# manikya7022/Continual-Learning-for-Dynamic-Video-Quality-Enhancement

Hardware: AMD Instinct MI355X
Metric: train frames/sec (2x SR, T=3, 540p->1080p) (higher is better)
Workload: dtype bf16

## Files before the change

### continual-learning-for-dynamic-video-quality-enhancement_amd/csrc/corr_mfma.hip

```cpp
#include <type_traits>
#include "common.h"

namespace nvq {

constexpr int MT_H = 8, MT_W = 16;
constexpr int MD = 4, MN = 9;
constexpr int MHH = MT_H + 2 * MD;
constexpr int MHW = MT_W + 2 * MD;
constexpr int MHP = MHH * MHW;
constexpr int M_T = 512;
constexpr int M_DSTR = 96;
constexpr int M_OSTR = 84;

typedef unsigned m_u32x4 __attribute__((ext_vector_type(4)));
typedef short m_s16x4 __attribute__((ext_vector_type(4)));

__device__ __forceinline__ unsigned pack_bf16x2(float lo, float hi) {
    typedef __bf16 b2 __attribute__((ext_vector_type(2)));
    const b2 v = {(__bf16)lo, (__bf16)hi};
    return __builtin_bit_cast(unsigned, v);
}
__device__ __forceinline__ m_u32x4 cvt_f8_bf16(float4 a, float4 b) {
    return (m_u32x4){pack_bf16x2(a.x, a.y), pack_bf16x2(a.z, a.w), pack_bf16x2(b.x, b.y), pack_bf16x2(b.z, b.w)};
}

template <int C, int YS>
__device__ __forceinline__ void m_stage_halo(const float* __restrict__ src, int ld, int n, int H, int W, int ty0, int tx0,
                                             __bf16* ys, int src_bf16) {
    constexpr int PPP = C / 8;
    constexpr int ITEMS = MHP * PPP;
    constexpr int PER = ITEMS / M_T;
    static_assert(ITEMS % M_T == 0, "halo pieces must divide evenly");
    if (src_bf16) {
        const __bf16* s16 = reinterpret_cast<const __bf16*>(src);
        m_u32x4 v[PER];
        unsigned okm = 0;
#pragma unroll
        for (int k = 0; k < PER; ++k) {
            const int item = threadIdx.x + k * M_T;
            const int hp = item / PPP, q = item - hp * PPP;
            const int hy = hp / MHW, hx = hp - hy * MHW;
            const int gy = ty0 + hy - MD, gx = tx0 + hx - MD;
            const bool ok = gy >= 0 && gy < H && gx >= 0 && gx < W;
            okm |= (ok ? 1u : 0u) << k;
            v[k] = *reinterpret_cast<const m_u32x4*>(s16 + (ok ? ((size_t)(n * H + gy) * W + gx) * ld + 8 * q : 0));
        }
#pragma unroll
        for (int k = 0; k < PER; ++k) {
            const int item = threadIdx.x + k * M_T;
            const int hp = item / PPP, q = item - hp * PPP;
            *reinterpret_cast<m_u32x4*>(ys + hp * YS + 8 * q) = (okm >> k) & 1 ? v[k] : (m_u32x4){0u, 0u, 0u, 0u};
        }
        return;
    }
    float4 a[PER], b[PER];
    unsigned okm = 0;
#pragma unroll
    for (int k = 0; k < PER; ++k) {
        const int item = threadIdx.x + k * M_T;
        const int hp = item / PPP, q = item - hp * PPP;
        const int hy = hp / MHW, hx = hp - hy * MHW;
        const int gy = ty0 + hy - MD, gx = tx0 + hx - MD;
        const bool ok = gy >= 0 && gy < H && gx >= 0 && gx < W;
        okm |= (ok ? 1u : 0u) << k;
        const float* p = src + (ok ? ((size_t)(n * H + gy) * W + gx) * ld + 8 * q : 0);
        a[k] = ld4(p);
        b[k] = ld4(p + 4);
    }
#pragma unroll
    for (int k = 0; k < PER; ++k) {
        const int item = threadIdx.x + k * M_T;
        const int hp = item / PPP, q = item - hp * PPP;
        const m_u32x4 v = cvt_f8_bf16(a[k], b[k]);
        *reinterpret_cast<m_u32x4*>(ys + hp * YS + 8 * q) = (okm >> k) & 1 ? v : (m_u32x4){0u, 0u, 0u, 0u};
    }
}

template <int C, bool OUT_BF16>
__global__ __launch_bounds__(M_T) void corr_fwd_mfma_kernel(const float* __restrict__ x1, int x1_ld,
                                                            const float* __restrict__ x2, int x2_ld, int x2_images, int H,
                                                            int W, int tilesX, int tilesY, float* __restrict__ out,
                                                            int out_ld, int in_bf16) {
    constexpr int YS = OUT_BF16 ? C + 8 : C + 16;
    constexpr int KS = C / 32;
    typedef typename std::conditional<OUT_BF16, __bf16, float>::type stage_t;
    __shared__ __attribute__((aligned(16))) __bf16 ys[MHP * YS];
    __shared__ __attribute__((aligned(16))) stage_t stage[MT_H * MT_W * M_OSTR];
    int bt = xcd_tile(blockIdx.x, gridDim.x);
    const int tx = bt % tilesX; bt /= tilesX;
    const int ty = bt % tilesY;
    const int n = bt / tilesY;
    const int lane = threadIdx.x & 63, r = threadIdx.x >> 6;
    const int p = lane & 15, g = lane >> 4;
    const int gy = ty * MT_H + r, gx = tx * MT_W + p;
    const bool inside = gy < H && gx < W;

    bf16x8 xb[KS];
    {
        const size_t off = inside ? ((size_t)(n * H + gy) * W + gx) * x1_ld : 0;
#pragma unroll
        for (int s = 0; s < KS; ++s) {
            if (in_bf16) {
                m_u32x4 v = *reinterpret_cast<const m_u32x4*>(reinterpret_cast<const __bf16*>(x1) + off + 32 * s + 8 * g);
                if (!inside) v = (m_u32x4){0u, 0u, 0u, 0u};
                xb[s] = __builtin_bit_cast(bf16x8, v);
            } else {
                float4 a = ld4(x1 + off + 32 * s + 8 * g), b = ld4(x1 + off + 32 * s + 8 * g + 4);
                if (!inside) { a = make_float4(0.f, 0.f, 0.f, 0.f); b = a; }
                xb[s] = __builtin_bit_cast(bf16x8, cvt_f8_bf16(a, b));
            }
        }
    }
    m_stage_halo<C, YS>(x2, x2_ld, n % x2_images, H, W, ty * MT_H, tx * MT_W, ys, in_bf16);
    stage_t* srow = stage + (r * MT_W) * M_OSTR;
    if (lane < 16) { srow[lane * M_OSTR + 81] = (stage_t)0.f; srow[lane * M_OSTR + 82] = (stage_t)0.f; srow[lane * M_OSTR + 83] = (stage_t)0.f; }
    __syncthreads();

    const float inv = 1.f / (float)C;
#pragma unroll 1
    for (int i = 0; i < MN; ++i) {
#pragma unroll
        for (int qb = 0; qb < 2; ++qb) {
            f32x4 acc = {0.f, 0.f, 0.f, 0.f};
            const __bf16* arow = ys + ((r + i) * MHW + qb * 8 + p) * YS + 8 * g;
#pragma unroll
            for (int s = 0; s < KS; ++s)
                acc = __builtin_amdgcn_mfma_f32_16x16x32_bf16(*reinterpret_cast<const bf16x8*>(arow + 32 * s), xb[s], acc, 0,
                                                              0, 0);
#pragma unroll
            for (int e = 0; e < 4; ++e) {
                const int m = 4 * g + e;
                const int j = qb * 8 + m - p;
                if (j >= 0 && j <= 8 && (qb == 0 || m >= 8)) srow[p * M_OSTR + i * MN + j] = (stage_t)(acc[e] * inv);
            }
        }
    }
    __syncthreads();
    if (gy >= H) return;
    if constexpr (OUT_BF16) {
        __bf16* o16 = reinterpret_cast<__bf16*>(out);
        const int ppp = out_ld / 8;
        for (int item = lane; item < MT_W * ppp; item += 64) {
            const int px = item / ppp, q = item - px * ppp;
            if (tx * MT_W + px >= W) continue;
            typedef unsigned u2 __attribute__((ext_vector_type(2)));
            u2 lo = {0u, 0u}, hi = {0u, 0u};
            if (8 * q < M_OSTR) lo = *reinterpret_cast<const u2*>(srow + px * M_OSTR + 8 * q);
            if (8 * q + 4 < M_OSTR) hi = *reinterpret_cast<const u2*>(srow + px * M_OSTR + 8 * q + 4);
            *reinterpret_cast<m_u32x4*>(o16 + ((size_t)(n * H + gy) * W + tx * MT_W + px) * out_ld + 8 * q) =
                (m_u32x4){lo[0], lo[1], hi[0], hi[1]};
        }
    } else {
        const int ppp = out_ld / 4;
        for (int item = lane; item < MT_W * ppp; item += 64) {
            const int px = item / ppp, q = item - px * ppp;
            if (tx * MT_W + px >= W) continue;
            float4 v = make_float4(0.f, 0.f, 0.f, 0.f);
            if (4 * q < M_OSTR) v = ld4(srow + px * M_OSTR + 4 * q);
            st4(out + ((size_t)(n * H + gy) * W + tx * MT_W + px) * out_ld + 4 * q, v);
        }
    }
}

constexpr int MS_SEG = 4;
constexpr int MS_MAXWG = 512;

template <int C, bool OUT_BF16>
__global__ __launch_bounds__(M_T) void corr_fwd_strip_kernel(const __bf16* __restrict__ x1, int x1_ld,
                                                             const __bf16* __restrict__ x2, int x2_ld, int x2_images, int H,
                                                             int W, int tilesX, int tilesY, int njobs,
                                                             float* __restrict__ out, int out_ld) {
    constexpr int YS = OUT_BF16 ? C + 8 : C + 16;
    constexpr int KS = C / 32;
    constexpr int PPP = C / 8;
    constexpr int HITEMS = 8 * MHW * PPP;
    constexpr int HPER = (HITEMS + M_T - 1) / M_T;
    typedef typename std::conditional<OUT_BF16, __bf16, float>::type stage_t;
    __shared__ __attribute__((aligned(16))) __bf16 ys[MHP * YS];
    __shared__ __attribute__((aligned(16))) stage_t stage[MT_H * MT_W * M_OSTR];
    const int tid = threadIdx.x;
    const int lane = tid & 63, r = tid >> 6;
    const int p = lane & 15, g = lane >> 4;
    stage_t* srow = stage + (r * MT_W) * M_OSTR;
    if (lane < 16) { srow[lane * M_OSTR + 81] = (stage_t)0.f; srow[lane * M_OSTR + 82] = (stage_t)0.f; srow[lane * M_OSTR + 83] = (stage_t)0.f; }
    const float inv = 1.f / (float)C;
    const int seg_rows = (tilesY + MS_SEG - 1) / MS_SEG;

    m_u32x4 hv[HPER], xv[KS];
    unsigned hokm = 0;
    bool xin = false;
    auto fetch_rows = [&](int n2, int ty, int tx, int half) {
        hokm = 0;
        int tid_o = tid;
        asm volatile("" : "+v"(tid_o));
#pragma unroll
        for (int k = 0; k < HPER; ++k) {
            const int item = tid_o + k * M_T;
            const int hp = item / PPP, q = item - hp * PPP;
            const int hyl = hp / MHW, hx = hp - hyl * MHW;
            const int gy = ty * MT_H + 8 * half + hyl - MD, gx = tx * MT_W + hx - MD;
            const bool ok = item < HITEMS && gy >= 0 && gy < H && gx >= 0 && gx < W;
            hokm |= (ok ? 1u : 0u) << k;
            hv[k] = *reinterpret_cast<const m_u32x4*>(x2 + (ok ? ((size_t)(n2 * H + gy) * W + gx) * x2_ld + 8 * q : 0));
        }
    };
    auto commit_rows = [&](int ty, int half) {
#pragma unroll
        for (int k = 0; k < HPER; ++k) {
            const int item = tid + k * M_T;
            const int hp = item / PPP, q = item - hp * PPP;
            const int hyl = hp / MHW, hx = hp - hyl * MHW;
            const int slot = (8 * half + hyl + 8 * (ty & 1)) & 15;
            if (item < HITEMS)
                *reinterpret_cast<m_u32x4*>(ys + (slot * MHW + hx) * YS + 8 * q) = (hokm >> k) & 1 ? hv[k] : (m_u32x4){0u, 0u, 0u, 0u};
        }
    };
    auto fetch_x1 = [&](int n, int ty, int tx) {
        const int gy = ty * MT_H + r, gx = tx * MT_W + p;
        xin = gy < H && gx < W;
        const size_t off = xin ? ((size_t)(n * H + gy) * W + gx) * x1_ld : 0;
#pragma unroll
        for (int s2 = 0; s2 < KS; ++s2) xv[s2] = *reinterpret_cast<const m_u32x4*>(x1 + off + 32 * s2 + 8 * g);
    };

    for (int job = blockIdx.x; job < njobs; job += gridDim.x) {
        int jt = job;
        const int seg = jt % MS_SEG; jt /= MS_SEG;
        const int tx = jt % tilesX;
        const int n = jt / tilesX;
        const int n2 = n % x2_images;
        const int ty0 = seg * seg_rows, ty1 = min(ty0 + seg_rows, tilesY);
        if (ty0 >= ty1) continue;
        __syncthreads();
        fetch_rows(n2, ty0, tx, 0);
        commit_rows(ty0, 0);
        fetch_rows(n2, ty0, tx, 1);
        fetch_x1(n, ty0, tx);
        for (int ty = ty0; ty < ty1; ++ty) {
            bf16x8 xb[KS];
            commit_rows(ty, 1);
#pragma unroll
            for (int s2 = 0; s2 < KS; ++s2) xb[s2] = __builtin_bit_cast(bf16x8, xin ? xv[s2] : (m_u32x4){0u, 0u, 0u, 0u});
            __syncthreads();
            if (ty + 1 < ty1) { fetch_rows(n2, ty + 1, tx, 1); fetch_x1(n, ty + 1, tx); }
            const int rot = 8 * (ty & 1);
#pragma unroll 1
            for (int i = 0; i < MN; ++i) {
#pragma unroll
                for (int qb = 0; qb < 2; ++qb) {
                    f32x4 acc = {0.f, 0.f, 0.f, 0.f};
                    const __bf16* arow = ys + ((((r + i) + rot) & 15) * MHW + qb * 8 + p) * YS + 8 * g;
#pragma unroll
                    for (int s2 = 0; s2 < KS; ++s2)
                        acc = __builtin_amdgcn_mfma_f32_16x16x32_bf16(*reinterpret_cast<const bf16x8*>(arow + 32 * s2), xb[s2], acc,
                                                                      0, 0, 0);
#pragma unroll
                    for (int e = 0; e < 4; ++e) {
                        const int m = 4 * g + e;
                        const int j = qb * 8 + m - p;
                        if (j >= 0 && j <= 8 && (qb == 0 || m >= 8)) srow[p * M_OSTR + i * MN + j] = (stage_t)(acc[e] * inv);
                    }
                }
            }
            const int gy = ty * MT_H + r;
            if (gy < H) {
                if constexpr (OUT_BF16) {
                    __bf16* o16 = reinterpret_cast<__bf16*>(out);
                    const int ppp = out_ld / 8;
                    for (int item = lane; item < MT_W * ppp; item += 64) {
                        const int px = item / ppp, q = item - px * ppp;
                        if (tx * MT_W + px >= W) continue;
                        typedef unsigned u2 __attribute__((ext_vector_type(2)));
                        u2 lo = {0u, 0u}, hi = {0u, 0u};
                        if (8 * q < M_OSTR) lo = *reinterpret_cast<const u2*>(srow + px * M_OSTR + 8 * q);
                        if (8 * q + 4 < M_OSTR) hi = *reinterpret_cast<const u2*>(srow + px * M_OSTR + 8 * q + 4);
                        *reinterpret_cast<m_u32x4*>(o16 + ((size_t)(n * H + gy) * W + tx * MT_W + px) * out_ld + 8 * q) =
                            (m_u32x4){lo[0], lo[1], hi[0], hi[1]};
                    }
                } else {
                    const int ppp = out_ld / 4;
                    for (int item = lane; item < MT_W * ppp; item += 64) {
                        const int px = item / ppp, q = item - px * ppp;
                        if (tx * MT_W + px >= W) continue;
                        float4 v = make_float4(0.f, 0.f, 0.f, 0.f);
                        if (4 * q < M_OSTR) v = ld4(srow + px * M_OSTR + 4 * q);
                        st4(out + ((size_t)(n * H + gy) * W + tx * MT_W + px) * out_ld + 4 * q, v);
                    }
                }
            }
            __syncthreads();
        }
    }
}

template <int C, int WHICH, bool D_BF16>
__global__ __launch_bounds__(M_T) void corr_bwd_mfma_kernel(const float* __restrict__ dcorr, int dcorr_ld,
                                                            const float* __restrict__ other, int other_ld,
                                                            int other_images, int H, int W, int tilesX, int tilesY,
                                                            float* __restrict__ dx, int dx_ld, int dx_coff,
                                                            int accumulate, int other_bf16, int groups, int group_images,
                                                            __bf16* __restrict__ dx16, int dx16_ld, const nvq_corr_addends ad) {
    constexpr int YS = WHICH == 1 ? C + 8 : C + 16;
    constexpr int NCB = C / 16;
    constexpr int DPX = WHICH == 1 ? MT_H * MT_W : MHP;
    __shared__ __attribute__((aligned(16))) __bf16 ys[MHP * YS];
    __shared__ __attribute__((aligned(16))) __bf16 ds[DPX * M_DSTR];
    int bt = xcd_tile(blockIdx.x, gridDim.x);
    const int tx = bt % tilesX; bt /= tilesX;
    const int ty = bt % tilesY;
    const int n0 = bt / tilesY;
    const int lane = threadIdx.x & 63, r = threadIdx.x >> 6;
    const int p = lane & 15, g = lane >> 4;
    f32x4 acc[NCB];
#pragma unroll
    for (int cb = 0; cb < NCB; ++cb) acc[cb] = (f32x4){0.f, 0.f, 0.f, 0.f};
#pragma unroll 1
    for (int gi = 0; gi < groups; ++gi) {
    const int n = n0 + gi * group_images;
    if (gi > 0) __syncthreads();

    {
        constexpr int ITEMS = DPX * 12;
        constexpr int PER = (ITEMS + M_T - 1) / M_T;
        const __bf16* d16 = reinterpret_cast<const __bf16*>(dcorr);
        if constexpr (D_BF16) {
            m_u32x4 v[PER];
            unsigned okm = 0;
#pragma unroll
            for (int k = 0; k < PER; ++k) {
                const int item = threadIdx.x + k * M_T;
                const int dp = item / 12, q = item - dp * 12;
                int gy, gx;
                if (WHICH == 1) { gy = ty * MT_H + dp / MT_W; gx = tx * MT_W + dp % MT_W; }
                else { gy = ty * MT_H + dp / MHW - MD; gx = tx * MT_W + dp % MHW - MD; }
                const bool ok = item < ITEMS && gy >= 0 && gy < H && gx >= 0 && gx < W;
                okm |= (ok ? 1u : 0u) << k;
                v[k] = *reinterpret_cast<const m_u32x4*>(d16 + (ok ? ((size_t)(n * H + gy) * W + gx) * dcorr_ld + 8 * q : 0));
            }
#pragma unroll
            for (int k = 0; k < PER; ++k) {
                const int item = threadIdx.x + k * M_T;
                const int dp = item / 12, q = item - dp * 12;
                if (item < ITEMS)
                    *reinterpret_cast<m_u32x4*>(ds + dp * M_DSTR + 8 * q) = (okm >> k) & 1 ? v[k] : (m_u32x4){0u, 0u, 0u, 0u};
            }
        } else {
#pragma unroll 3
            for (int k = 0; k < PER; ++k) {
                const int item = threadIdx.x + k * M_T;
                if (item >= ITEMS) break;
                const int dp = item / 12, q = item - dp * 12;
                int gy, gx;
                if (WHICH == 1) { gy = ty * MT_H + dp / MT_W; gx = tx * MT_W + dp % MT_W; }
                else { gy = ty * MT_H + dp / MHW - MD; gx = tx * MT_W + dp % MHW - MD; }
                const bool ok = gy >= 0 && gy < H && gx >= 0 && gx < W;
                m_u32x4 v = {0u, 0u, 0u, 0u};
                if (ok) {
                    const size_t idx = ((size_t)(n * H + gy) * W + gx) * dcorr_ld + 8 * q;
                    v = cvt_f8_bf16(ld4(dcorr + idx), ld4(dcorr + idx + 4));
                }
                *reinterpret_cast<m_u32x4*>(ds + dp * M_DSTR + 8 * q) = v;
            }
        }
    }
    m_stage_halo<C, YS>(other, other_ld, n % other_images, H, W, ty * MT_H, tx * MT_W, ys, other_bf16);
    __syncthreads();

    typedef m_s16x4 __attribute__((address_space(3))) * lds_tr_ptr;
    const int trq = p >> 2, trp = p & 3;
    const int gq = g < 3 ? g : 2;
    const unsigned short* dsu = reinterpret_cast<const unsigned short*>(ds);
#pragma unroll 1
    for (int i = 0; i < MN; ++i) {
        unsigned bw[4];
#pragma unroll
        for (int t2 = 0; t2 < 4; ++t2) {
            unsigned half[2];
#pragma unroll
            for (int h = 0; h < 2; ++h) {
                const int q = 8 * g + 2 * t2 + h;
                const int j = q - p;
                const bool band = j >= 0 && j <= 8;
                int idx;
                if (WHICH == 1) idx = (r * MT_W + p) * M_DSTR + i * MN + (band ? j : 0);
                else idx = ((r + i) * MHW + (band ? q : 0)) * M_DSTR + (8 - i) * MN + (band ? 8 - j : 0);
                const unsigned v = dsu[idx];
                half[h] = band ? v : 0u;
            }
            bw[t2] = half[0] | (half[1] << 16);
        }
        const bf16x8 bfrag = __builtin_bit_cast(bf16x8, (m_u32x4){bw[0], bw[1], bw[2], bw[3]});
        const __bf16* yrow = ys + ((r + i) * MHW + 8 * gq + trq) * YS + 4 * trp;
#pragma unroll
        for (int cb = 0; cb < NCB; ++cb) {
            const m_s16x4 a0 = __builtin_amdgcn_ds_read_tr16_b64_v4i16((lds_tr_ptr)(yrow + cb * 16));
            const m_s16x4 a1 = __builtin_amdgcn_ds_read_tr16_b64_v4i16((lds_tr_ptr)(yrow + 4 * YS + cb * 16));
            typedef short s16x8 __attribute__((ext_vector_type(8)));
            const s16x8 a = {a0[0], a0[1], a0[2], a0[3], a1[0], a1[1], a1[2], a1[3]};
            acc[cb] = __builtin_amdgcn_mfma_f32_16x16x32_bf16(__builtin_bit_cast(bf16x8, a), bfrag, acc[cb], 0, 0, 0);
        }
    }
    }
    const int gy = ty * MT_H + r, gx = tx * MT_W + p;
    if (gy >= H || gx >= W) return;
    const float inv = 1.f / (float)C;
    float* op = dx + ((size_t)(n0 * H + gy) * W + gx) * dx_ld + dx_coff + 4 * g;
    float4 old[NCB];
    if (accumulate) {
#pragma unroll
        for (int cb = 0; cb < NCB; ++cb) old[cb] = ld4(op + cb * 16);
    }
    typedef unsigned u2_t __attribute__((ext_vector_type(2)));
    u2_t ra[NCB], rb[NCB];
    const size_t apix = (size_t)(n0 * H + gy) * W + gx;
    if (ad.a) {
#pragma unroll
        for (int cb = 0; cb < NCB; ++cb)
            ra[cb] = *reinterpret_cast<const u2_t*>(reinterpret_cast<const __bf16*>(ad.a) + apix * ad.a_ld + ad.a_coff + cb * 16 + 4 * g);
    }
    if (ad.b) {
#pragma unroll
        for (int cb = 0; cb < NCB; ++cb)
            rb[cb] = *reinterpret_cast<const u2_t*>(reinterpret_cast<const __bf16*>(ad.b) + apix * ad.b_ld + ad.b_coff + cb * 16 + 4 * g);
    }
    auto add_raw = [](float4& v, u2_t w) {
        v.x += __uint_as_float(w[0] << 16); v.y += __uint_as_float(w[0] & 0xffff0000u);
        v.z += __uint_as_float(w[1] << 16); v.w += __uint_as_float(w[1] & 0xffff0000u);
    };
#pragma unroll
    for (int cb = 0; cb < NCB; ++cb) {
        float4 v = make_float4(acc[cb][0] * inv, acc[cb][1] * inv, acc[cb][2] * inv, acc[cb][3] * inv);
        if (accumulate) { v.x += old[cb].x; v.y += old[cb].y; v.z += old[cb].z; v.w += old[cb].w; }
        if (ad.a) add_raw(v, ra[cb]);
        if (ad.b) add_raw(v, rb[cb]);
        if (dx16)
            *reinterpret_cast<bf16x4*>(dx16 + ((size_t)(n0 * H + gy) * W + gx) * dx16_ld + cb * 16 + 4 * g) =
                (bf16x4){(__bf16)v.x, (__bf16)v.y, (__bf16)v.z, (__bf16)v.w};
        else
            st4(op + cb * 16, v);
    }
}

template <int C>
__global__ __launch_bounds__(M_T) void corr_bwd1_strip_kernel(const __bf16* __restrict__ dcorr, int dcorr_ld,
                                                              const __bf16* __restrict__ other, int other_ld, int other_images,
                                                              int H, int W, int tilesX, int tilesY, int njobs,
                                                              float* __restrict__ dx, int dx_ld, int dx_coff, int accumulate,
                                                              __bf16* __restrict__ dx16, int dx16_ld, const nvq_corr_addends ad) {
    constexpr int YS = C + 8;
    constexpr int NCB = C / 16;
    constexpr int PPP = C / 8;
    constexpr int HITEMS = 8 * MHW * PPP;
    constexpr int HPER = (HITEMS + M_T - 1) / M_T;
    constexpr int DITEMS = MT_H * MT_W * 12;
    constexpr int DPER = (DITEMS + M_T - 1) / M_T;
    __shared__ __attribute__((aligned(16))) __bf16 ys[MHP * YS];
    __shared__ __attribute__((aligned(16))) __bf16 ds[MT_H * MT_W * M_DSTR];
    const int tid = threadIdx.x;
    const int lane = tid & 63, r = tid >> 6;
    const int p = lane & 15, g = lane >> 4;
    const int seg_rows = (tilesY + MS_SEG - 1) / MS_SEG;
    const float inv = 1.f / (float)C;

    m_u32x4 hv[HPER], dv[DPER];
    unsigned hokm = 0, dokm = 0;
    auto fetch_rows = [&](int n2, int ty, int tx, int half) {
        hokm = 0;
        int tid_o = tid;
        asm volatile("" : "+v"(tid_o));
#pragma unroll
        for (int k = 0; k < HPER; ++k) {
            const int item = tid_o + k * M_T;
            const int hp = item / PPP, q = item - hp * PPP;
            const int hyl = hp / MHW, hx = hp - hyl * MHW;
            const int gy = ty * MT_H + 8 * half + hyl - MD, gx = tx * MT_W + hx - MD;
            const bool ok = item < HITEMS && gy >= 0 && gy < H && gx >= 0 && gx < W;
            hokm |= (ok ? 1u : 0u) << k;
            hv[k] = *reinterpret_cast<const m_u32x4*>(other + (ok ? ((size_t)(n2 * H + gy) * W + gx) * other_ld + 8 * q : 0));
        }
    };
    auto commit_rows = [&](int ty, int half) {
#pragma unroll
        for (int k = 0; k < HPER; ++k) {
            const int item = tid + k * M_T;
            const int hp = item / PPP, q = item - hp * PPP;
            const int hyl = hp / MHW, hx = hp - hyl * MHW;
            const int slot = (8 * half + hyl + 8 * (ty & 1)) & 15;
            if (item < HITEMS)
                *reinterpret_cast<m_u32x4*>(ys + (slot * MHW + hx) * YS + 8 * q) = (hokm >> k) & 1 ? hv[k] : (m_u32x4){0u, 0u, 0u, 0u};
        }
    };
    auto fetch_d = [&](int n, int ty, int tx) {
        dokm = 0;
        int tid_o = tid;
        asm volatile("" : "+v"(tid_o));
#pragma unroll
        for (int k = 0; k < DPER; ++k) {
            const int item = tid_o + k * M_T;
            const int dp = item / 12, q = item - dp * 12;
            const int gy = ty * MT_H + dp / MT_W, gx = tx * MT_W + dp % MT_W;
            const bool ok = item < DITEMS && gy < H && gx < W;
            dokm |= (ok ? 1u : 0u) << k;
            dv[k] = *reinterpret_cast<const m_u32x4*>(dcorr + (ok ? ((size_t)(n * H + gy) * W + gx) * dcorr_ld + 8 * q : 0));
        }
    };
    auto commit_d = [&]() {
#pragma unroll
        for (int k = 0; k < DPER; ++k) {
            const int item = tid + k * M_T;
            const int dp = item / 12, q = item - dp * 12;
            if (item < DITEMS)
                *reinterpret_cast<m_u32x4*>(ds + dp * M_DSTR + 8 * q) = (dokm >> k) & 1 ? dv[k] : (m_u32x4){0u, 0u, 0u, 0u};
        }
    };
    typedef m_s16x4 __attribute__((address_space(3))) * lds_tr_ptr;
    const int trq = p >> 2, trp = p & 3;
    const int gq = g < 3 ? g : 2;
    const unsigned short* dsu = reinterpret_cast<const unsigned short*>(ds);

    for (int job = blockIdx.x; job < njobs; job += gridDim.x) {
        int jt = job;
        const int seg = jt % MS_SEG; jt /= MS_SEG;
        const int tx = jt % tilesX;
        const int n = jt / tilesX;
        const int n2 = n % other_images;
        const int ty0 = seg * seg_rows, ty1 = min(ty0 + seg_rows, tilesY);
        if (ty0 >= ty1) continue;
        __syncthreads();
        fetch_rows(n2, ty0, tx, 0);
        commit_rows(ty0, 0);
        fetch_rows(n2, ty0, tx, 1);
        fetch_d(n, ty0, tx);
        for (int ty = ty0; ty < ty1; ++ty) {
            commit_rows(ty, 1);
            commit_d();
            __syncthreads();
            if (ty + 1 < ty1) { fetch_rows(n2, ty + 1, tx, 1); fetch_d(n, ty + 1, tx); }
            const int rot = 8 * (ty & 1);
            f32x4 acc[NCB];
#pragma unroll
            for (int cb = 0; cb < NCB; ++cb) acc[cb] = (f32x4){0.f, 0.f, 0.f, 0.f};
#pragma unroll 1
            for (int i = 0; i < MN; ++i) {
                unsigned bw[4];
#pragma unroll
                for (int t2 = 0; t2 < 4; ++t2) {
                    unsigned half[2];
#pragma unroll
                    for (int h = 0; h < 2; ++h) {
                        const int q = 8 * g + 2 * t2 + h;
                        const int j = q - p;
                        const bool band = j >= 0 && j <= 8;
                        const unsigned v = dsu[(r * MT_W + p) * M_DSTR + i * MN + (band ? j : 0)];
                        half[h] = band ? v : 0u;
                    }
                    bw[t2] = half[0] | (half[1] << 16);
                }
                const bf16x8 bfrag = __builtin_bit_cast(bf16x8, (m_u32x4){bw[0], bw[1], bw[2], bw[3]});
                const __bf16* yrow = ys + ((((r + i) + rot) & 15) * MHW + 8 * gq + trq) * YS + 4 * trp;
#pragma unroll
                for (int cb = 0; cb < NCB; ++cb) {
                    const m_s16x4 a0 = __builtin_amdgcn_ds_read_tr16_b64_v4i16((lds_tr_ptr)(yrow + cb * 16));
                    const m_s16x4 a1 = __builtin_amdgcn_ds_read_tr16_b64_v4i16((lds_tr_ptr)(yrow + 4 * YS + cb * 16));
                    typedef short s16x8 __attribute__((ext_vector_type(8)));
                    const s16x8 a = {a0[0], a0[1], a0[2], a0[3], a1[0], a1[1], a1[2], a1[3]};
                    acc[cb] = __builtin_amdgcn_mfma_f32_16x16x32_bf16(__builtin_bit_cast(bf16x8, a), bfrag, acc[cb], 0, 0, 0);
                }
            }
            const int gy = ty * MT_H + r, gx = tx * MT_W + p;
            if (gy < H && gx < W) {
                const size_t apix = (size_t)(n * H + gy) * W + gx;
                float* op = dx + apix * dx_ld + dx_coff + 4 * g;
                float4 old[NCB];
                if (accumulate) {
#pragma unroll
                    for (int cb = 0; cb < NCB; ++cb) old[cb] = ld4(op + cb * 16);
                }
                typedef unsigned u2_t __attribute__((ext_vector_type(2)));
                u2_t ra[NCB], rb[NCB];
                if (ad.a) {
#pragma unroll
                    for (int cb = 0; cb < NCB; ++cb)
                        ra[cb] = *reinterpret_cast<const u2_t*>(reinterpret_cast<const __bf16*>(ad.a) + apix * ad.a_ld + ad.a_coff + cb * 16 + 4 * g);
                }
                if (ad.b) {
#pragma unroll
                    for (int cb = 0; cb < NCB; ++cb)
                        rb[cb] = *reinterpret_cast<const u2_t*>(reinterpret_cast<const __bf16*>(ad.b) + apix * ad.b_ld + ad.b_coff + cb * 16 + 4 * g);
                }
                auto add_raw = [](float4& v, u2_t w) {
                    v.x += __uint_as_float(w[0] << 16); v.y += __uint_as_float(w[0] & 0xffff0000u);
                    v.z += __uint_as_float(w[1] << 16); v.w += __uint_as_float(w[1] & 0xffff0000u);
                };
#pragma unroll
                for (int cb = 0; cb < NCB; ++cb) {
                    float4 v = make_float4(acc[cb][0] * inv, acc[cb][1] * inv, acc[cb][2] * inv, acc[cb][3] * inv);
                    if (accumulate) { v.x += old[cb].x; v.y += old[cb].y; v.z += old[cb].z; v.w += old[cb].w; }
                    if (ad.a) add_raw(v, ra[cb]);
                    if (ad.b) add_raw(v, rb[cb]);
                    if (dx16)
                        *reinterpret_cast<bf16x4*>(dx16 + apix * dx16_ld + cb * 16 + 4 * g) =
                            (bf16x4){(__bf16)v.x, (__bf16)v.y, (__bf16)v.z, (__bf16)v.w};
                    else
                        st4(op + cb * 16, v);
                }
            }
            __syncthreads();
        }
    }
}

template <int C>
__global__ __launch_bounds__(M_T) void corr_bwd2_pf_kernel(const __bf16* __restrict__ dcorr, int dcorr_ld,
                                                           const __bf16* __restrict__ other, int other_ld, int other_images,
                                                           int H, int W, int tilesX, int tilesY, int ntiles,
                                                           float* __restrict__ dx, int dx_ld, int dx_coff, int accumulate,
                                                           int groups, int group_images, __bf16* __restrict__ dx16, int dx16_ld,
                                                           const nvq_corr_addends ad) {
    constexpr int YS = C + 16;
    constexpr int NCB = C / 16;
    constexpr int PPP = C / 8;
    constexpr int YITEMS = MHP * PPP, YPER = YITEMS / M_T;
    constexpr int DITEMS = MHP * 12, DPER = DITEMS / M_T;
    static_assert(YITEMS % M_T == 0 && DITEMS % M_T == 0, "halo pieces divide evenly");
    __shared__ __attribute__((aligned(16))) __bf16 ys[MHP * YS];
    __shared__ __attribute__((aligned(16))) __bf16 ds[MHP * M_DSTR];
    const int tid = threadIdx.x;
    const int lane = tid & 63, r = tid >> 6;
    const int p = lane & 15, g = lane >> 4;
    const float inv = 1.f / (float)C;

    m_u32x4 yv[YPER], dv[DPER];
    unsigned yokm = 0, dokm = 0;
    auto locate = [&](int tile, int& n0, int& ty, int& tx) {
        int bt = xcd_tile(tile, ntiles);
        tx = bt % tilesX; bt /= tilesX;
        ty = bt % tilesY;
        n0 = bt / tilesY;
    };
    auto fetch = [&](int n, int ty, int tx) {
        yokm = 0; dokm = 0;
        int tid_o = tid;
        asm volatile("" : "+v"(tid_o));
        const int n2 = n % other_images;
#pragma unroll
        for (int k = 0; k < YPER; ++k) {
            const int item = tid_o + k * M_T;
            const int hp = item / PPP, q = item - hp * PPP;
            const int hy = hp / MHW, hx = hp - hy * MHW;
            const int gy = ty * MT_H + hy - MD, gx = tx * MT_W + hx - MD;
            const bool ok = gy >= 0 && gy < H && gx >= 0 && gx < W;
            yokm |= (ok ? 1u : 0u) << k;
            yv[k] = *reinterpret_cast<const m_u32x4*>(other + (ok ? ((size_t)(n2 * H + gy) * W + gx) * other_ld + 8 * q : 0));
        }
#pragma unroll
        for (int k = 0; k < DPER; ++k) {
            const int item = tid_o + k * M_T;
            const int dp = item / 12, q = item - dp * 12;
            const int gy = ty * MT_H + dp / MHW - MD, gx = tx * MT_W + dp % MHW - MD;
            const bool ok = gy >= 0 && gy < H && gx >= 0 && gx < W;
            dokm |= (ok ? 1u : 0u) << k;
            dv[k] = *reinterpret_cast<const m_u32x4*>(dcorr + (ok ? ((size_t)(n * H + gy) * W + gx) * dcorr_ld + 8 * q : 0));
        }
    };
    auto commit = [&]() {
#pragma unroll
        for (int k = 0; k < YPER; ++k) {
            const int item = tid + k * M_T;
            const int hp = item / PPP, q = item - hp * PPP;
            *reinterpret_cast<m_u32x4*>(ys + hp * YS + 8 * q) = (yokm >> k) & 1 ? yv[k] : (m_u32x4){0u, 0u, 0u, 0u};
        }
#pragma unroll
        for (int k = 0; k < DPER; ++k) {
            const int item = tid + k * M_T;
            const int dp = item / 12, q = item - dp * 12;
            *reinterpret_cast<m_u32x4*>(ds + dp * M_DSTR + 8 * q) = (dokm >> k) & 1 ? dv[k] : (m_u32x4){0u, 0u, 0u, 0u};
        }
    };
    typedef m_s16x4 __attribute__((address_space(3))) * lds_tr_ptr;
    const int trq = p >> 2, trp = p & 3;
    const int gq = g < 3 ? g : 2;
    const unsigned short* dsu = reinterpret_cast<const unsigned short*>(ds);

    int tile = blockIdx.x;
    if (tile < ntiles) { int n0, ty, tx; locate(tile, n0, ty, tx); fetch(n0, ty, tx); }
    for (; tile < ntiles; tile += gridDim.x) {
        int n0, ty, tx;
        locate(tile, n0, ty, tx);
        f32x4 acc[NCB];
#pragma unroll
        for (int cb = 0; cb < NCB; ++cb) acc[cb] = (f32x4){0.f, 0.f, 0.f, 0.f};
#pragma unroll 1
        for (int gi = 0; gi < groups; ++gi) {
            __syncthreads();
            commit();
            __syncthreads();
            if (gi + 1 < groups) {
                fetch(n0 + (gi + 1) * group_images, ty, tx);
            } else if (tile + (int)gridDim.x < ntiles) {
                int n1, ty1, tx1;
                locate(tile + gridDim.x, n1, ty1, tx1);
                fetch(n1, ty1, tx1);
            }
#pragma unroll 1
            for (int i = 0; i < MN; ++i) {
                unsigned bw[4];
#pragma unroll
                for (int t2 = 0; t2 < 4; ++t2) {
                    unsigned half[2];
#pragma unroll
                    for (int h = 0; h < 2; ++h) {
                        const int q = 8 * g + 2 * t2 + h;
                        const int j = q - p;
                        const bool band = j >= 0 && j <= 8;
                        const unsigned v = dsu[((r + i) * MHW + (band ? q : 0)) * M_DSTR + (8 - i) * MN + (band ? 8 - j : 0)];
                        half[h] = band ? v : 0u;
                    }
                    bw[t2] = half[0] | (half[1] << 16);
                }
                const bf16x8 bfrag = __builtin_bit_cast(bf16x8, (m_u32x4){bw[0], bw[1], bw[2], bw[3]});
                const __bf16* yrow = ys + ((r + i) * MHW + 8 * gq + trq) * YS + 4 * trp;
#pragma unroll
                for (int cb = 0; cb < NCB; ++cb) {
                    const m_s16x4 a0 = __builtin_amdgcn_ds_read_tr16_b64_v4i16((lds_tr_ptr)(yrow + cb * 16));
                    const m_s16x4 a1 = __builtin_amdgcn_ds_read_tr16_b64_v4i16((lds_tr_ptr)(yrow + 4 * YS + cb * 16));
                    typedef short s16x8 __attribute__((ext_vector_type(8)));
                    const s16x8 a = {a0[0], a0[1], a0[2], a0[3], a1[0], a1[1], a1[2], a1[3]};
                    acc[cb] = __builtin_amdgcn_mfma_f32_16x16x32_bf16(__builtin_bit_cast(bf16x8, a), bfrag, acc[cb], 0, 0, 0);
                }
            }
        }
        const int gy = ty * MT_H + r, gx = tx * MT_W + p;
        if (gy < H && gx < W) {
            const size_t apix = (size_t)(n0 * H + gy) * W + gx;
            float* op = dx + apix * dx_ld + dx_coff + 4 * g;
            float4 old[NCB];
            if (accumulate) {
#pragma unroll
                for (int cb = 0; cb < NCB; ++cb) old[cb] = ld4(op + cb * 16);
            }
            typedef unsigned u2_t __attribute__((ext_vector_type(2)));
            u2_t ra[NCB], rb[NCB];
            if (ad.a) {
#pragma unroll
                for (int cb = 0; cb < NCB; ++cb)
                    ra[cb] = *reinterpret_cast<const u2_t*>(reinterpret_cast<const __bf16*>(ad.a) + apix * ad.a_ld + ad.a_coff + cb * 16 + 4 * g);
            }
            if (ad.b) {
#pragma unroll
                for (int cb = 0; cb < NCB; ++cb)
                    rb[cb] = *reinterpret_cast<const u2_t*>(reinterpret_cast<const __bf16*>(ad.b) + apix * ad.b_ld + ad.b_coff + cb * 16 + 4 * g);
            }
            auto add_raw = [](float4& v, u2_t w) {
                v.x += __uint_as_float(w[0] << 16); v.y += __uint_as_float(w[0] & 0xffff0000u);
                v.z += __uint_as_float(w[1] << 16); v.w += __uint_as_float(w[1] & 0xffff0000u);
            };
#pragma unroll
            for (int cb = 0; cb < NCB; ++cb) {
                float4 v = make_float4(acc[cb][0] * inv, acc[cb][1] * inv, acc[cb][2] * inv, acc[cb][3] * inv);
                if (accumulate) { v.x += old[cb].x; v.y += old[cb].y; v.z += old[cb].z; v.w += old[cb].w; }
                if (ad.a) add_raw(v, ra[cb]);
                if (ad.b) add_raw(v, rb[cb]);
                if (dx16)
                    *reinterpret_cast<bf16x4*>(dx16 + apix * dx16_ld + cb * 16 + 4 * g) =
                        (bf16x4){(__bf16)v.x, (__bf16)v.y, (__bf16)v.z, (__bf16)v.w};
                else
                    st4(op + cb * 16, v);
            }
        }
    }
}

bool corr_mfma_supported(int C) { return C == 32 || C == 64; }

int corr_forward_mfma(const float* x1, int x1_ld, const float* x2, int x2_ld, int x2_images, int C, int N, int H, int W,
                      float* out, int out_ld, int out_bf16, int in_bf16, hipStream_t s) {
    NVQ_REQUIRE(!in_bf16 || (x1_ld % 8 == 0 && x2_ld % 8 == 0), "correlation_forward(bf16): bf16 inputs need ld %% 8 == 0");
    NVQ_REQUIRE(out_ld >= 84 && out_ld % (out_bf16 ? 8 : 4) == 0, "correlation_forward(bf16): out_ld %d", out_ld);
    const int tilesX = (W + MT_W - 1) / MT_W, tilesY = (H + MT_H - 1) / MT_H;
    if (in_bf16) {
        const int njobs = N * tilesX * MS_SEG;
        int nwg = njobs < MS_MAXWG ? njobs : MS_MAXWG;
#define NVQ_CS(CC, OB) \
    hipLaunchKernelGGL((corr_fwd_strip_kernel<CC, OB>), dim3(nwg), dim3(M_T), 0, s, reinterpret_cast<const __bf16*>(x1), x1_ld, \
                       reinterpret_cast<const __bf16*>(x2), x2_ld, x2_images, H, W, tilesX, tilesY, njobs, out, out_ld)
        if (C == 64) { if (out_bf16) NVQ_CS(64, true); else NVQ_CS(64, false); }
        else { if (out_bf16) NVQ_CS(32, true); else NVQ_CS(32, false); }
#undef NVQ_CS
        return check_launch("correlation_forward(bf16, strip)");
    }
    const dim3 grid((unsigned)((long)tilesX * tilesY * N));
#define NVQ_CF(CC, OB) \
    hipLaunchKernelGGL((corr_fwd_mfma_kernel<CC, OB>), grid, dim3(M_T), 0, s, x1, x1_ld, x2, x2_ld, x2_images, H, W, tilesX, tilesY, out, out_ld, in_bf16)
    if (C == 64) { if (out_bf16) NVQ_CF(64, true); else NVQ_CF(64, false); }
    else { if (out_bf16) NVQ_CF(32, true); else NVQ_CF(32, false); }
#undef NVQ_CF
    return check_launch("correlation_forward(bf16)");
}

int corr_backward_mfma(int which, const float* dcorr, int dcorr_ld, int dcorr_bf16, const float* other, int other_ld,
                       int other_images, int C, int N, int H, int W, float* dx, int dx_ld, int dx_coff, int accumulate,
                       int other_bf16, int groups, float* dx16, int dx16_ld, const nvq_corr_addends* addends, hipStream_t s) {
    const nvq_corr_addends ad = addends ? *addends : nvq_corr_addends{nullptr, 0, 0, nullptr, 0, 0};
    NVQ_REQUIRE((!ad.a || (ad.a_ld % 4 == 0 && ad.a_coff % 4 == 0 && (reinterpret_cast<uintptr_t>(ad.a) & 7) == 0)) &&
                    (!ad.b || (ad.b_ld % 4 == 0 && ad.b_coff % 4 == 0 && (reinterpret_cast<uintptr_t>(ad.b) & 7) == 0)),
                "correlation_backward(bf16): addends need 8-byte aligned rows");
    NVQ_REQUIRE(!other_bf16 || other_ld % 8 == 0, "correlation_backward(bf16): a bf16 `other` needs ld %% 8 == 0");
    NVQ_REQUIRE(dcorr_ld >= 96 && dcorr_ld % (dcorr_bf16 ? 8 : 4) == 0,
                "correlation_backward(bf16): dcorr must be readable up to channel 96 (ld %d)", dcorr_ld);
    const int tilesX = (W + MT_W - 1) / MT_W, tilesY = (H + MT_H - 1) / MT_H;
    if (which == 1 && dcorr_bf16 && other_bf16 && dcorr_ld % 8 == 0) {
        const int njobs = N * tilesX * MS_SEG;
        const int nwg = njobs < MS_MAXWG ? njobs : MS_MAXWG;
#define NVQ_CB1(CC) hipLaunchKernelGGL(corr_bwd1_strip_kernel<CC>, dim3(nwg), dim3(M_T), 0, s, reinterpret_cast<const __bf16*>(dcorr), \
                                       dcorr_ld, reinterpret_cast<const __bf16*>(other), other_ld, other_images, H, W, tilesX, tilesY, \
                                       njobs, dx, dx_ld, dx_coff, accumulate, reinterpret_cast<__bf16*>(dx16), dx16_ld, ad)
        if (C == 64) NVQ_CB1(64); else NVQ_CB1(32);
#undef NVQ_CB1
        return check_launch("correlation_backward(bf16, strip)");
    }
    if (which == 2 && dcorr_bf16 && other_bf16 && dcorr_ld % 8 == 0) {
        const int ntiles = tilesX * tilesY * N;
        int nwg = ntiles < 256 ? ntiles : 256;
        if (nwg >= 8) nwg &= ~7;
#define NVQ_CB2P(CC) hipLaunchKernelGGL(corr_bwd2_pf_kernel<CC>, dim3(nwg), dim3(M_T), 0, s, reinterpret_cast<const __bf16*>(dcorr), \
                                        dcorr_ld, reinterpret_cast<const __bf16*>(other), other_ld, other_images, H, W, tilesX, tilesY, \
                                        ntiles, dx, dx_ld, dx_coff, accumulate, groups, N, reinterpret_cast<__bf16*>(dx16), dx16_ld, ad)
        if (C == 64) NVQ_CB2P(64); else NVQ_CB2P(32);
#undef NVQ_CB2P
        return check_launch("correlation_backward(bf16, prefetching)");
    }
    const dim3 grid((unsigned)((long)tilesX * tilesY * N));
#define NVQ_CB(CC, WH, DB) \
    hipLaunchKernelGGL((corr_bwd_mfma_kernel<CC, WH, DB>), grid, dim3(M_T), 0, s, dcorr, dcorr_ld, other, other_ld, other_images, H, W, tilesX, tilesY, dx, dx_ld, dx_coff, accumulate, other_bf16, groups, N, reinterpret_cast<__bf16*>(dx16), dx16_ld, ad)
#define NVQ_CB2(CC) \
    do { if (which == 1) { if (dcorr_bf16) NVQ_CB(CC, 1, true); else NVQ_CB(CC, 1, false); } \
         else { if (dcorr_bf16) NVQ_CB(CC, 2, true); else NVQ_CB(CC, 2, false); } } while (0)
    if (C == 64) NVQ_CB2(64); else NVQ_CB2(32);
#undef NVQ_CB2
#undef NVQ_CB
    return check_launch("correlation_backward(bf16)");
}

}
```

Before: 78.05.

## Prefetch epilogue addends early, precompute halo descriptors, and stage only needed dcorr rows

Measured after the change: 78.40, median of 6. No clear change (+0.4%).

```diff
diff --git a/continual-learning-for-dynamic-video-quality-enhancement_amd/csrc/corr_mfma.hip b/continual-learning-for-dynamic-video-quality-enhancement_amd/csrc/corr_mfma.hip
--- a/continual-learning-for-dynamic-video-quality-enhancement_amd/csrc/corr_mfma.hip
+++ b/continual-learning-for-dynamic-video-quality-enhancement_amd/csrc/corr_mfma.hip
@@ -1,15 +1,9 @@
 #include <type_traits>
 #include "common.h"
+#include "corr_stage_map.h"
 
 namespace nvq {
 
-constexpr int MT_H = 8, MT_W = 16;
-constexpr int MD = 4, MN = 9;
-constexpr int MHH = MT_H + 2 * MD;
-constexpr int MHW = MT_W + 2 * MD;
-constexpr int MHP = MHH * MHW;
-constexpr int M_T = 512;
-constexpr int M_DSTR = 96;
 constexpr int M_OSTR = 84;
 
 typedef unsigned m_u32x4 __attribute__((ext_vector_type(4)));
@@ -22,6 +16,18 @@
 }
 __device__ __forceinline__ m_u32x4 cvt_f8_bf16(float4 a, float4 b) {
     return (m_u32x4){pack_bf16x2(a.x, a.y), pack_bf16x2(a.z, a.w), pack_bf16x2(b.x, b.y), pack_bf16x2(b.z, b.w)};
+}
+
+typedef unsigned m_u32x2 __attribute__((ext_vector_type(2)));
+template <int N>
+__device__ __forceinline__ void m_arrived(const m_u32x2 (&v)[N]) {
+#pragma unroll
+    for (int k = 0; k < N; ++k) asm volatile("" ::"v"(v[k]));
+}
+template <int N>
+__device__ __forceinline__ void m_arrived(const float4 (&v)[N]) {
+#pragma unroll
+    for (int k = 0; k < N; ++k) asm volatile("" ::"v"(v[k].x), "v"(v[k].y), "v"(v[k].z), "v"(v[k].w));
 }
 
 template <int C, int YS>
@@ -536,6 +542,25 @@
             commit_d();
             __syncthreads();
             if (ty + 1 < ty1) { fetch_rows(n2, ty + 1, tx, 1); fetch_d(n, ty + 1, tx); }
+            const int gy = ty * MT_H + r, gx = tx * MT_W + p;
+            const bool inside = gy < H && gx < W;
+            const size_t apix = inside ? (size_t)(n * H + gy) * W + gx : 0;
+            float* op = dx + apix * dx_ld + dx_coff + 4 * g;
+            typedef unsigned u2_t __attribute__((ext_vector_type(2)));
+            float4 old[NCB];
+            u2_t ra[NCB], rb[NCB];
+            {
+                const float* po = accumulate ? op : reinterpret_cast<const float*>(dcorr);
+                const int so = accumulate ? 16 : 0;
+                const __bf16* pa = ad.a ? reinterpret_cast<const __bf16*>(ad.a) + apix * ad.a_ld + ad.a_coff + 4 * g : dcorr;
+                const __bf16* pb = ad.b ? reinterpret_cast<const __bf16*>(ad.b) + apix * ad.b_ld + ad.b_coff + 4 * g : dcorr;
+#pragma unroll
+                for (int cb = 0; cb < NCB; ++cb) {
+                    old[cb] = ld4(po + cb * so);
+                    ra[cb] = *reinterpret_cast<const u2_t*>(pa + cb * 16);
+                    rb[cb] = *reinterpret_cast<const u2_t*>(pb + cb * 16);
+                }
+            }
             const int rot = 8 * (ty & 1);
             f32x4 acc[NCB];
 #pragma unroll
@@ -567,27 +592,8 @@
                     acc[cb] = __builtin_amdgcn_mfma_f32_16x16x32_bf16(__builtin_bit_cast(bf16x8, a), bfrag, acc[cb], 0, 0, 0);
                 }
             }
-            const int gy = ty * MT_H + r, gx = tx * MT_W + p;
-            if (gy < H && gx < W) {
-                const size_t apix = (size_t)(n * H + gy) * W + gx;
-                float* op = dx + apix * dx_ld + dx_coff + 4 * g;
-                float4 old[NCB];
-                if (accumulate) {
-#pragma unroll
-                    for (int cb = 0; cb < NCB; ++cb) old[cb] = ld4(op + cb * 16);
-                }
-                typedef unsigned u2_t __attribute__((ext_vector_type(2)));
-                u2_t ra[NCB], rb[NCB];
-                if (ad.a) {
-#pragma unroll
-                    for (int cb = 0; cb < NCB; ++cb)
-                        ra[cb] = *reinterpret_cast<const u2_t*>(reinterpret_cast<const __bf16*>(ad.a) + apix * ad.a_ld + ad.a_coff + cb * 16 + 4 * g);
-                }
-                if (ad.b) {
-#pragma unroll
-                    for (int cb = 0; cb < NCB; ++cb)
-                        rb[cb] = *reinterpret_cast<const u2_t*>(reinterpret_cast<const __bf16*>(ad.b) + apix * ad.b_ld + ad.b_coff + cb * 16 + 4 * g);
-                }
+            m_arrived(old); m_arrived(ra); m_arrived(rb);
+            if (inside) {
                 auto add_raw = [](float4& v, u2_t w) {
                     v.x += __uint_as_float(w[0] << 16); v.y += __uint_as_float(w[0] & 0xffff0000u);
                     v.z += __uint_as_float(w[1] << 16); v.w += __uint_as_float(w[1] & 0xffff0000u);
@@ -621,8 +627,8 @@
     constexpr int NCB = C / 16;
     constexpr int PPP = C / 8;
     constexpr int YITEMS = MHP * PPP, YPER = YITEMS / M_T;
-    constexpr int DITEMS = MHP * 12, DPER = DITEMS / M_T;
-    static_assert(YITEMS % M_T == 0 && DITEMS % M_T == 0, "halo pieces divide evenly");
+    constexpr int DPER = X2G_DPER;
+    static_assert(YITEMS % M_T == 0, "halo pieces divide evenly");
     __shared__ __attribute__((aligned(16))) __bf16 ys[MHP * YS];
     __shared__ __attribute__((aligned(16))) __bf16 ds[MHP * M_DSTR];
     const int tid = threadIdx.x;
@@ -638,29 +644,42 @@
         ty = bt % tilesY;
         n0 = bt / tilesY;
     };
+    unsigned ydesc[YPER], ddesc[DPER];
+#pragma unroll
+    for (int k = 0; k < YPER; ++k) {
+        const int item = tid + k * M_T;
+        const int hp = item / PPP, q = item - hp * PPP;
+        const int hy = hp / MHW, hx = hp - hy * MHW;
+        ydesc[k] = (unsigned)hy | (unsigned)hx << 8 | (unsigned)q << 16;
+    }
+#pragma unroll
+    for (int k = 0; k < DPER; ++k) {
+        const x2g_piece d = x2g_dcorr_item(tid + k * M_T);
+        ddesc[k] = (unsigned)d.hy | (unsigned)d.hx << 8 | (unsigned)d.piece << 16 | (d.valid ? 1u << 24 : 0u);
+    }
     auto fetch = [&](int n, int ty, int tx) {
         yokm = 0; dokm = 0;
-        int tid_o = tid;
-        asm volatile("" : "+v"(tid_o));
         const int n2 = n % other_images;
 #pragma unroll
         for (int k = 0; k < YPER; ++k) {
-            const int item = tid_o + k * M_T;
-            const int hp = item / PPP, q = item - hp * PPP;
-            const int hy = hp / MHW, hx = hp - hy * MHW;
-            const int gy = ty * MT_H + hy - MD, gx = tx * MT_W + hx - MD;
-            const bool ok = gy >= 0 && gy < H && gx >= 0 && gx < W;
+            unsigned e = ydesc[k];
+            asm volatile("" : "+v"(e));
+            const int hy = e & 255, hx = (e >> 8) & 255, q = e >> 16;
+            int gy, gx;
+            const bool ok = corr_halo_pixel(ty, tx, hy, hx, H, W, gy, gx);
             yokm |= (ok ? 1u : 0u) << k;
             yv[k] = *reinterpret_cast<const m_u32x4*>(other + (ok ? ((size_t)(n2 * H + gy) * W + gx) * other_ld + 8 * q : 0));
         }
 #pragma unroll
         for (int k = 0; k < DPER; ++k) {
-            const int item = tid_o + k * M_T;
-            const int dp = item / 12, q = item - dp * 12;
-            const int gy = ty * MT_H + dp / MHW - MD, gx = tx * MT_W + dp % MHW - MD;
-            const bool ok = gy >= 0 && gy < H && gx >= 0 && gx < W;
+            unsigned e = ddesc[k];
+            asm volatile("" : "+v"(e));
+            x2g_piece d;
+            d.hy = e & 255; d.hx = (e >> 8) & 255; d.piece = (e >> 16) & 255; d.valid = e >> 24;
+            int gy, gx;
+            const bool ok = corr_halo_pixel(ty, tx, d.hy, d.hx, H, W, gy, gx) && d.valid;
             dokm |= (ok ? 1u : 0u) << k;
-            dv[k] = *reinterpret_cast<const m_u32x4*>(dcorr + (ok ? ((size_t)(n * H + gy) * W + gx) * dcorr_ld + 8 * q : 0));
+            dv[k] = *reinterpret_cast<const m_u32x4*>(dcorr + (ok ? ((size_t)(n * H + gy) * W + gx) * dcorr_ld + 8 * d.piece : 0));
         }
     };
     auto commit = [&]() {
@@ -672,9 +691,9 @@
         }
 #pragma unroll
         for (int k = 0; k < DPER; ++k) {
-            const int item = tid + k * M_T;
-            const int dp = item / 12, q = item - dp * 12;
-            *reinterpret_cast<m_u32x4*>(ds + dp * M_DSTR + 8 * q) = (dokm >> k) & 1 ? dv[k] : (m_u32x4){0u, 0u, 0u, 0u};
+            const x2g_piece d = x2g_dcorr_item(tid + k * M_T);
+            if (d.valid)
+                *reinterpret_cast<m_u32x4*>(ds + x2g_ds_piece_offset(d)) = (dokm >> k) & 1 ? dv[k] : (m_u32x4){0u, 0u, 0u, 0u};
         }
     };
     typedef m_s16x4 __attribute__((address_space(3))) * lds_tr_ptr;
@@ -690,19 +709,38 @@
         f32x4 acc[NCB];
 #pragma unroll
         for (int cb = 0; cb < NCB; ++cb) acc[cb] = (f32x4){0.f, 0.f, 0.f, 0.f};
-#pragma unroll 1
-        for (int gi = 0; gi < groups; ++gi) {
+        const int gy = ty * MT_H + r, gx = tx * MT_W + p;
+        const bool inside = gy < H && gx < W;
+        const size_t apix = inside ? (size_t)(n0 * H + gy) * W + gx : 0;
+        float* op = dx + apix * dx_ld + dx_coff + 4 * g;
+        typedef unsigned u2_t __attribute__((ext_vector_type(2)));
+        float4 old[NCB];
+        u2_t ra[NCB], rb[NCB];
+        auto step = [&](int gi, auto last_c) {
+            constexpr bool LAST = decltype(last_c)::value;
             __syncthreads();
             commit();
             __syncthreads();
-            if (gi + 1 < groups) {
+            if constexpr (!LAST) {
                 fetch(n0 + (gi + 1) * group_images, ty, tx);
             } else if (tile + (int)gridDim.x < ntiles) {
                 int n1, ty1, tx1;
                 locate(tile + gridDim.x, n1, ty1, tx1);
                 fetch(n1, ty1, tx1);
             }
-#pragma unroll 1
+            if constexpr (LAST) {
+                const float* po = accumulate ? op : reinterpret_cast<const float*>(dcorr);
+                const int so = accumulate ? 16 : 0;
+                const __bf16* pa = ad.a ? reinterpret_cast<const __bf16*>(ad.a) + apix * ad.a_ld + ad.a_coff + 4 * g : dcorr;
+                const __bf16* pb = ad.b ? reinterpret_cast<const __bf16*>(ad.b) + apix * ad.b_ld + ad.b_coff + 4 * g : dcorr;
+#pragma unroll
+                for (int cb = 0; cb < NCB; ++cb) {
+                    old[cb] = ld4(po + cb * so);
+                    ra[cb] = *reinterpret_cast<const u2_t*>(pa + cb * 16);
+                    rb[cb] = *reinterpret_cast<const u2_t*>(pb + cb * 16);
+                }
+            }
+#pragma unroll
             for (int i = 0; i < MN; ++i) {
                 unsigned bw[4];
 #pragma unroll
@@ -710,10 +748,8 @@
                     unsigned half[2];
 #pragma unroll
                     for (int h = 0; h < 2; ++h) {
-                        const int q = 8 * g + 2 * t2 + h;
-                        const int j = q - p;
-                        const bool band = j >= 0 && j <= 8;
-                        const unsigned v = dsu[((r + i) * MHW + (band ? q : 0)) * M_DSTR + (8 - i) * MN + (band ? 8 - j : 0)];
+                        bool band;
+                        const unsigned v = dsu[x2g_band_half(r, i, 8 * g + 2 * t2 + h, p, band)];
                         half[h] = band ? v : 0u;
                     }
                     bw[t2] = half[0] | (half[1] << 16);
@@ -729,28 +765,12 @@
                     acc[cb] = __builtin_amdgcn_mfma_f32_16x16x32_bf16(__builtin_bit_cast(bf16x8, a), bfrag, acc[cb], 0, 0, 0);
                 }
             }
-        }
-        const int gy = ty * MT_H + r, gx = tx * MT_W + p;
-        if (gy < H && gx < W) {
-            const size_t apix = (size_t)(n0 * H + gy) * W + gx;
-            float* op = dx + apix * dx_ld + dx_coff + 4 * g;
-            float4 old[NCB];
-            if (accumulate) {
-#pragma unroll
-                for (int cb = 0; cb < NCB; ++cb) old[cb] = ld4(op + cb * 16);
-            }
-            typedef unsigned u2_t __attribute__((ext_vector_type(2)));
-            u2_t ra[NCB], rb[NCB];
-            if (ad.a) {
-#pragma unroll
-                for (int cb = 0; cb < NCB; ++cb)
-                    ra[cb] = *reinterpret_cast<const u2_t*>(reinterpret_cast<const __bf16*>(ad.a) + apix * ad.a_ld + ad.a_coff + cb * 16 + 4 * g);
-            }
-            if (ad.b) {
-#pragma unroll
-                for (int cb = 0; cb < NCB; ++cb)
-                    rb[cb] = *reinterpret_cast<const u2_t*>(reinterpret_cast<const __bf16*>(ad.b) + apix * ad.b_ld + ad.b_coff + cb * 16 + 4 * g);
-            }
+        };
+#pragma unroll 1
+        for (int gi = 0; gi + 1 < groups; ++gi) step(gi, std::false_type());
+        step(groups - 1, std::true_type());
+        m_arrived(old); m_arrived(ra); m_arrived(rb);
+        if (inside) {
             auto add_raw = [](float4& v, u2_t w) {
                 v.x += __uint_as_float(w[0] << 16); v.y += __uint_as_float(w[0] & 0xffff0000u);
                 v.z += __uint_as_float(w[1] << 16); v.w += __uint_as_float(w[1] & 0xffff0000u);
diff --git a/continual-learning-for-dynamic-video-quality-enhancement_amd/csrc/corr_stage_map.h b/continual-learning-for-dynamic-video-quality-enhancement_amd/csrc/corr_stage_map.h
--- /dev/null
+++ b/continual-learning-for-dynamic-video-quality-enhancement_amd/csrc/corr_stage_map.h
@@ -0,0 +1,67 @@
+#pragma once
+
+#if defined(__HIPCC__) || defined(__CUDACC__)
+#define NVQ_MAP_HD __host__ __device__ inline __attribute__((always_inline))
+#else
+#define NVQ_MAP_HD inline
+#endif
+
+namespace nvq {
+
+constexpr int MT_H = 8, MT_W = 16;
+constexpr int MD = 4, MN = 9;
+constexpr int MHH = MT_H + 2 * MD;
+constexpr int MHW = MT_W + 2 * MD;
+constexpr int MHP = MHH * MHW;
+constexpr int M_T = 512;
+constexpr int M_DSTR = 96;
+
+NVQ_MAP_HD void x2g_row_window(int hy, int& ch_lo, int& ch_hi) {
+    const int i_lo = hy - (MT_H - 1) > 0 ? hy - (MT_H - 1) : 0, i_hi = hy < MN - 1 ? hy : MN - 1;
+    ch_lo = (MN - 1 - i_hi) * MN;
+    ch_hi = (MN - 1 - i_lo) * MN + MN;
+}
+
+constexpr int X2G_SLOTS = 12;
+constexpr int X2G_DITEMS = MT_H * MHW * X2G_SLOTS;
+constexpr int X2G_DPER = (X2G_DITEMS + M_T - 1) / M_T;
+
+struct x2g_piece {
+    int hy, hx, piece;
+    bool valid;
+};
+
+NVQ_MAP_HD x2g_piece x2g_dcorr_item(int item) {
+    const int px = item / X2G_SLOTS, slot = item - px * X2G_SLOTS;
+    const int pair = px / MHW, hx = px - pair * MHW;
+    const int e = (MT_H - pair) * MN;
+    const int last_lo = (e - 1) >> 3;
+    x2g_piece d;
+    d.hx = hx;
+    if (slot <= last_lo) {
+        d.hy = pair + MT_H;
+        d.piece = slot;
+    } else {
+        d.hy = pair;
+        d.piece = slot - (last_lo + 1) + (e >> 3);
+    }
+    d.valid = item < X2G_DITEMS && d.piece <= (MN * MN - 1) / 8;
+    return d;
+}
+
+NVQ_MAP_HD int x2g_ds_piece_offset(const x2g_piece& d) { return (d.hy * MHW + d.hx) * M_DSTR + 8 * d.piece; }
+
+NVQ_MAP_HD int x2g_band_half(int r, int i, int q, int p, bool& band) {
+    const int j = q - p;
+    band = j >= 0 && j <= MN - 1;
+    return ((r + i) * MHW + (band ? q : 0)) * M_DSTR + (MN - 1 - i) * MN + (band ? MN - 1 - j : 0);
+}
+
+NVQ_MAP_HD int corr_tiles(int extent, int tile) { return (extent + tile - 1) / tile; }
+NVQ_MAP_HD bool corr_halo_pixel(int ty, int tx, int hy, int hx, int H, int W, int& gy, int& gx) {
+    gy = ty * MT_H + hy - MD;
+    gx = tx * MT_W + hx - MD;
+    return gy >= 0 && gy < H && gx >= 0 && gx < W;
+}
+
+}
```
